# jw007123/hp-Adaptive-Signed-Distance-Field-Octree

Hardware: AMD Instinct MI355X
Metric: Query() Mpts/sec at targetError=1e-5 (union3 field, 10M SplitMix64 pts per GPU, HBM-resident); Create() ms reported as create_ms (higher is better)
Workload: dtype f64

## Files before the change

### hp-adaptive-signed-distance-field-octree_amd/csrc/fit_analytic.hip

```cpp
#include "fit_kernels.hpp"

namespace hpsdf {

HPSDF_FIT_KIND_UNIT(, kFieldAnalytic)

}
```

### hp-adaptive-signed-distance-field-octree_amd/csrc/fit_kernels.hpp

```cpp
#pragma once
#include <hip/hip_runtime.h>

#include <cstdint>

#include "device_types.hpp"
#include "field_glue.hpp"
#include "launch.hpp"

namespace hpsdf {


constexpr int kFitPiece = 8;
#ifndef HPSDF_FIT_MIN_WAVES
#define HPSDF_FIT_MIN_WAVES 4
#endif

__device__ __forceinline__ double fitRowAny(double acc, double a1, const double* __restrict__ tk, double n2,
                                            const double* __restrict__ F, int nq) {
    int k = 0;
    for (; k + 4 <= nq; k += 4) {
        const double f0 = F[k], f1 = F[k + 1], f2 = F[k + 2], f3 = F[k + 3];
        const double t0 = tk[k], t1 = tk[k + 1], t2 = tk[k + 2], t3 = tk[k + 3];
        acc = acc + (a1 * t0 * n2) * f0;
        acc = acc + (a1 * t1 * n2) * f1;
        acc = acc + (a1 * t2 * n2) * f2;
        acc = acc + (a1 * t3 * n2) * f3;
    }
    for (; k < nq; ++k) acc = acc + (a1 * tk[k] * n2) * F[k];
    return acc;
}

template <int KIND, bool CSG, int DEG, int R, bool LEFT>
__device__ __forceinline__ void fitBlockBody(const FitBlock blk, const FitTask* __restrict__ tasks, double* __restrict__ arena,
                                             double* __restrict__ errs, double* __restrict__ mirror,
                                             const DeviceTables* __restrict__ T, const FieldDev& field, const RootMap& rm, double* lds) {
    static_assert(R == 1 || DEG > 0, "cell blocking needs a compile-time degree");
    __shared__ double sNl[13 * 11];
    __shared__ double sRec[26];
    __shared__ int32_t sMeshStack[kFitThreads / 64][kMeshStack];
    __shared__ unsigned char sPosI[KIND == kFieldMesh ? 64 : 4], sPosJK[KIND == kFieldMesh ? 64 : 4];
    const int tid = threadIdx.x;
    const int deg = DEG > 0 ? DEG : (int)blk.degree;
    const int nq = 4 * deg + 1, nq2 = nq * nq, G = blk.nTasks;
    const int rowStart = blk.rowStart, rowEnd = blk.rowEnd, nrows = rowEnd - rowStart;
    const int gl = nq * (nq - 1) / 2;
    const int planes = blk.planesPerChunk;
    const int depth = blk.depth;
    const bool split = blk.split != 0;

    double* sT = lds;
    double* sR = sT + (deg + 1) * nq;
    double* sW = sR + nq;
    double* sC = sW + nq;
    double* sF = sC + 8 * G;

    stageQueryTables(T, sNl, sRec);
    for (int q = tid; q < nq; q += kFitThreads) {
        const double x = T->roots[gl + q];
        sR[q] = x;
        sW[q] = T->weights[gl + q];
        double m2 = 0.0, m1 = 1.0;
        sT[q] = 1.0;
        for (int i = 1; i <= deg; ++i) {
            const double l = T->rec[i][0] * x * m1 - T->rec[i][1] * m2;
            m2 = m1, m1 = l;
            sT[i * nq + q] = l;
        }
    }
    for (int g = tid; g < G; g += kFitThreads) {
        const FitTask& tk = tasks[blk.firstTask + g];
        double sc[3];
        for (int a = 0; a < 3; ++a) {
            sc[a] = (double)(tk.bmax[a] - tk.bmin[a]) * 0.5;
            sC[8 * g + 3 + a] = (double)((tk.bmin[a] + tk.bmax[a]) / 2.0f);
            sC[8 * g + a] = sc[a];
        }
        sC[8 * g + 6] = prod3<LEFT>(sc[0], sc[1], sc[2]);
        sC[8 * g + 7] = __longlong_as_double((long long)tk.sampleOff);
    }
    __syncthreads();

    const bool wide = DEG == 0 && nrows > kFitThreads;
    const int slot = wide ? 0 : tid / nrows;
    const int g2 = slot * R;
    const int r0 = rowStart + (wide ? tid : tid % nrows);
    const int r1 = r0 + kFitThreads;
    const bool act0 = wide ? (r0 < rowEnd) : (tid < ((G + R - 1) / R) * nrows);
    const bool act1 = wide && r1 < rowEnd;
    int i0a = 0, i1a = 0, i2a = 0, i0b = 0, i1b = 0, i2b = 0;
    double n0a = 0, n1a = 0, n2a = 0, n0b = 0, n1b = 0, n2b = 0;
    if (act0) {
        i0a = T->bidx[r0][0], i1a = T->bidx[r0][1], i2a = T->bidx[r0][2];
        n0a = sNl[i0a * 11 + depth], n1a = sNl[i1a * 11 + depth], n2a = sNl[i2a * 11 + depth];
    }
    if (act1) {
        i0b = T->bidx[r1][0], i1b = T->bidx[r1][1], i2b = T->bidx[r1][2];
        n0b = sNl[i0b * 11 + depth], n1b = sNl[i1b * 11 + depth], n2b = sNl[i2b * 11 + depth];
    }
    constexpr int NQF = DEG > 0 ? 4 * DEG + 1 : 1;
    double tkReg[NQF];
    if (DEG > 0) {
#pragma unroll
        for (int k = 0; k < NQF; ++k) tkReg[k] = sT[i2a * nq + k];
    }
    uint32_t meshHint = 0xFFFFFFFFu;
    double acc[R];
#pragma unroll
    for (int r = 0; r < R; ++r) acc[r] = 0.0;
    double acc1 = 0.0;

    const int cellStride = planes * nq2;
    for (int iBase = 0; iBase < nq; iBase += planes) {
        const int np = min(planes, nq - iBase);
        if constexpr (KIND == kFieldMesh) {
            if (tid < nq) {
                int rank = 0;
                for (int b = 0; b < nq; ++b) rank += sR[b] < sR[tid] ? 1 : 0;
                sPosJK[rank] = (unsigned char)tid;
            }
            if (tid >= 64 && tid < 64 + np) {
                const int a = tid - 64;
                int rank = 0;
                for (int b = 0; b < np; ++b) rank += sR[iBase + b] < sR[iBase + a] ? 1 : 0;
                sPosI[rank] = (unsigned char)a;
            }
            __syncthreads();
        }
        if constexpr (KIND != kFieldMesh) {
            const int cols = G * nq2;
            for (int c0 = 0; c0 < cols; c0 += kFitThreads) {
                const int cc = c0 + tid;
                const bool activeS = cc < cols;
                const int ccl = activeS ? cc : cols - 1;
                const int g = ccl / nq2, jk = ccl - g * nq2, j = jk / nq, k = jk - j * nq;
                const double* c = sC + 8 * g;
                const double uy = sR[j] * c[1] + c[4], uz = sR[k] * c[2] + c[5];
                const double wy = uy * rm.bounds[1] + rm.centre[1];
                const double wz = uz * rm.bounds[2] + rm.centre[2];
                const double wj = sW[j], wk = sW[k], c6 = c[6];
                const uint64_t sbase = (uint64_t)__double_as_longlong(c[7]) + (uint64_t)(j * nq + k);
                for (int il = 0; il < np; ++il) {
                    const int i = iBase + il;
                    const double ux = sR[i] * c[0] + c[3];
                    const double wx = ux * rm.bounds[0] + rm.centre[0];
                    const uint64_t sidx = sbase + (uint64_t)(i * nq2);
                    const double fv = activeS ? fieldEvalWorld<KIND, CSG, LEFT>(field, wx, wy, wz, sidx, sNl, sRec, meshHint) : 0.0;
                    if (activeS) {
                        sF[g * cellStride + il * nq2 + jk] = c6 * prod3<LEFT>(sW[i], wj, wk) * fv;
                        if (split) const_cast<double*>(field.samples)[sidx] = fv;
                    }
                }
            }
        } else {
            const int chunkSamples = np * nq2, total = G * chunkSamples;
            const float invChunk = 1.0f / (float)chunkSamples;
            for (int s0 = 0; s0 < total; s0 += kFitThreads) {
                const int s = s0 + tid;
                const bool activeS = s < total;
                const int sc = activeS ? s : total - 1;
                int g = (int)(((float)sc + 0.5f) * invChunk);
                int rem = sc - g * chunkSamples;
                if (rem < 0) {
                    --g;
                    rem += chunkSamples;
                } else if (rem >= chunkSamples) {
                    ++g;
                    rem -= chunkSamples;
                }
                if constexpr (KIND == kFieldMesh) rem = meshSampleOrder(rem, np, nq, sPosI, sPosJK);
                const double* c = sC + 8 * g;
                const int il = rem / nq2, jk = rem - il * nq2, j = jk / nq, k = jk - j * nq, i = iBase + il;
                const double ux = sR[i] * c[0] + c[3], uy = sR[j] * c[1] + c[4], uz = sR[k] * c[2] + c[5];
                const double wx = ux * rm.bounds[0] + rm.centre[0];
                const double wy = uy * rm.bounds[1] + rm.centre[1];
                const double wz = uz * rm.bounds[2] + rm.centre[2];
                const uint64_t sidx = (uint64_t)__double_as_longlong(c[7]) + (uint64_t)((i * nq + j) * nq + k);
                double fv;
                if constexpr (KIND == kFieldMesh) {
                    const double mv = (double)meshSignedDistanceWave(field.mesh, V3{(float)wx, (float)wy, (float)wz}, activeS, meshHint,
                                                                     sMeshStack[tid >> 6]);
                    fv = activeS ? applyCsg<CSG>(field, mv, wx, wy, wz, sNl, sRec) : 0.0;
                } else {
                    fv = activeS ? fieldEvalWorld<KIND, CSG, LEFT>(field, wx, wy, wz, sidx, sNl, sRec, meshHint) : 0.0;
                }
                if (activeS) {
                    sF[g * cellStride + rem] = c[6] * prod3<LEFT>(sW[i], sW[j], sW[k]) * fv;
                    if constexpr (KIND != kFieldMesh)
                        if (split) const_cast<double*>(field.samples)[sidx] = fv;
                }
            }
        }
        __syncthreads();
        if (act0) {
            const double* tj = sT + i1a * nq;
            const double* tk = sT + i2a * nq;
            for (int il = 0; il < np; ++il) {
                const double* F = sF + g2 * cellStride + il * nq2;
                const double a0 = sT[i0a * nq + iBase + il] * n0a;
#ifdef HPSDF_FIT_ROW_UNROLL
#pragma unroll HPSDF_FIT_ROW_UNROLL
#endif
                for (int j = 0; j < nq; ++j) {
                    const double a1 = a0 * tj[j] * n1a;
                    if constexpr (DEG > 0 && DEG <= 5) {
                        double lp[NQF];
#pragma unroll
                        for (int k = 0; k < NQF; ++k) lp[k] = a1 * tkReg[k] * n2a;
#pragma unroll
                        for (int r = 0; r < R; ++r) {
                            const double* Fr = F + r * cellStride + j * nq;
                            double f[NQF];
#pragma unroll
                            for (int k = 0; k < NQF; ++k) f[k] = Fr[k];
#pragma unroll
                            for (int k = 0; k < NQF; ++k) acc[r] = acc[r] + lp[k] * f[k];
                        }
                    } else if constexpr (DEG > 5) {
                        const double* Fr = F + j * nq;
#pragma unroll
                        for (int k0 = 0; k0 < NQF; k0 += kFitPiece) {
                            double lp[kFitPiece], f[kFitPiece];
#pragma unroll
                            for (int k = 0; k < kFitPiece; ++k)
                                if (k0 + k < NQF) f[k] = Fr[k0 + k];
#pragma unroll
                            for (int k = 0; k < kFitPiece; ++k)
                                if (k0 + k < NQF) lp[k] = a1 * tkReg[k0 + k] * n2a;
#pragma unroll
                            for (int k = 0; k < kFitPiece; ++k)
                                if (k0 + k < NQF) acc[0] = acc[0] + lp[k] * f[k];
                        }
                    } else {
                        acc[0] = fitRowAny(acc[0], a1, tk, n2a, F + j * nq, nq);
                    }
                }
            }
        }
        if (act1) {
            const double* tj = sT + i1b * nq;
            const double* tk = sT + i2b * nq;
            for (int il = 0; il < np; ++il) {
                const double* F = sF + il * nq2;
                const double a0 = sT[i0b * nq + iBase + il] * n0b;
                for (int j = 0; j < nq; ++j) {
                    const double a1 = a0 * tj[j] * n1b;
                    acc1 = fitRowAny(acc1, a1, tk, n2b, F + j * nq, nq);
                }
            }
        }
        __syncthreads();
    }

    const bool weighted = blk.weighted != 0;
    const int stashStride = weighted ? rowEnd : nrows, stashBase = weighted ? 0 : rowStart;
    const int outBase = split ? 0 : stashBase;
    if (act0) {
#pragma unroll
        for (int r = 0; r < R; ++r)
            if (g2 + r < G) {
                const uint64_t at = tasks[blk.firstTask + g2 + r].outOff + (r0 - outBase);
                arena[at] = acc[r];
                if (mirror != nullptr) mirror[at] = acc[r];
                sF[(g2 + r) * stashStride + (r0 - stashBase)] = acc[r];
            }
    }
    if (act1) {
        arena[tasks[blk.firstTask].outOff + (r1 - outBase)] = acc1;
        sF[r1 - stashBase] = acc1;
    }
    if (weighted && rowStart > 0) {
        for (int s = tid; s < G * rowStart; s += kFitThreads) {
            const int g = s / rowStart, r = s - g * rowStart;
            const FitTask& tk = tasks[blk.firstTask + g];
            const double v = arena[tk.copyOff + r];
            arena[tk.outOff + r] = v;
            sF[g * stashStride + r] = v;
        }
    }
    __syncthreads();
    for (int g = tid; g < G; g += kFitThreads) {
        const int first = deg > 0 ? (int)T->count[deg - 1] : 0;
        double e = 0.0;
        for (int r = first > rowStart ? first : rowStart; r < rowEnd; ++r)
            if (T->bidx[r][3] == deg) {
                const double c = sF[g * stashStride + (r - stashBase)];
                e = e + c * c;
            }
        errs[tasks[blk.firstTask + g].errSlot] = e;
    }
}

template <int KIND, bool CSG, bool LEFT>
__global__ __launch_bounds__(kFitThreads, HPSDF_FIT_MIN_WAVES) void fit_multi_kernel(const FitBlock* __restrict__ blocks,
                                                                const FitTask* __restrict__ tasks, double* __restrict__ arena,
                                                                double* __restrict__ errs, const DeviceTables* __restrict__ T,
                                                                FieldDev field, RootMap rm, const uint32_t* __restrict__ count,
                                                                uint32_t countValue) {
    extern __shared__ double lds[];
    const uint32_t n = count ? *count : countValue;
    if (blockIdx.x >= n) return;
    const FitBlock blk = blocks[n - 1u - blockIdx.x];
    switch (blk.degree) {
        case 2: fitBlockBody<KIND, CSG, 2, 1, LEFT>(blk, tasks, arena, errs, nullptr, T, field, rm, lds); break;
        case 3: fitBlockBody<KIND, CSG, 3, 1, LEFT>(blk, tasks, arena, errs, nullptr, T, field, rm, lds); break;
        case 4: fitBlockBody<KIND, CSG, 4, 1, LEFT>(blk, tasks, arena, errs, nullptr, T, field, rm, lds); break;
        case 5: fitBlockBody<KIND, CSG, 5, 1, LEFT>(blk, tasks, arena, errs, nullptr, T, field, rm, lds); break;
        case 6: fitBlockBody<KIND, CSG, 6, 1, LEFT>(blk, tasks, arena, errs, nullptr, T, field, rm, lds); break;
        case 7: fitBlockBody<KIND, CSG, 7, 1, LEFT>(blk, tasks, arena, errs, nullptr, T, field, rm, lds); break;
        case 8: fitBlockBody<KIND, CSG, 8, 1, LEFT>(blk, tasks, arena, errs, nullptr, T, field, rm, lds); break;
        default: fitBlockBody<KIND, CSG, 0, 1, LEFT>(blk, tasks, arena, errs, nullptr, T, field, rm, lds); break;
    }
}

template <int KIND, bool CSG, int DEG, int R, bool LEFT>
__global__ __launch_bounds__(kFitThreads, HPSDF_FIT_MIN_WAVES) void fit_kernel(const FitBlock* __restrict__ blocks,
                                                          const FitTask* __restrict__ tasks, double* __restrict__ arena,
                                                          double* __restrict__ errs, double* __restrict__ mirror,
                                                          const DeviceTables* __restrict__ T, FieldDev field, RootMap rm,
                                                          const uint32_t* __restrict__ range) {
    extern __shared__ double lds[];
    uint32_t b = blockIdx.x;
    if (range != nullptr) {
        if (b >= range[1]) return;
        b += range[0];
    }
    fitBlockBody<KIND, CSG, DEG, R, LEFT>(blocks[b], tasks, arena, errs, mirror, T, field, rm, lds);
}

template <int KIND, bool CSG, bool LEFT>
__global__ __launch_bounds__(256) void field_kernel(FieldDev f, const DeviceTables* __restrict__ T,
                                                    const double* __restrict__ xyz, size_t n, double* __restrict__ out) {
    __shared__ double sNl[13 * 11];
    __shared__ double sRec[26];
    stageQueryTables(T, sNl, sRec);
    __syncthreads();
    const size_t stride = (size_t)gridDim.x * blockDim.x;
    uint32_t hint = 0xFFFFFFFFu;
    for (size_t i = (size_t)blockIdx.x * blockDim.x + threadIdx.x; i < n; i += stride)
        out[i] = fieldEvalWorld<KIND, CSG, LEFT>(f, xyz[3 * i], xyz[3 * i + 1], xyz[3 * i + 2], i, sNl, sRec, hint);
}

template <int KIND, bool CSG, bool LEFT>
static void launchFitT(hipStream_t stream, int degree, int cellsPerThread, const FitBlock* dBlocks, uint32_t nBlocks,
                       size_t ldsBytes, const FitTask* dTasks, double* dArena, double* dErrs, double* dMeans,
                       const DeviceTables* dTables, const FieldDev& field, const RootMap& rm, const uint32_t* dRange) {
#define HPSDF_FIT_LAUNCH(D, RR)                                                                                       \
    hipLaunchKernelGGL((fit_kernel<KIND, CSG, D, RR, LEFT>), dim3(nBlocks), dim3(kFitThreads), ldsBytes, stream, dBlocks, \
                       dTasks, dArena, dErrs, dMeans, dTables, field, rm, dRange)
#define HPSDF_FIT_CASE(D)       \
    case D:                     \
        HPSDF_FIT_LAUNCH(D, 1); \
        break;
    if (cellsPerThread != 1 && cellsPerThread != 4) cellsPerThread = 1;
    switch (degree) {
        HPSDF_FIT_CASE(2)
        HPSDF_FIT_CASE(3)
        HPSDF_FIT_CASE(4)
        HPSDF_FIT_CASE(5)
        HPSDF_FIT_CASE(6)
        HPSDF_FIT_CASE(7)
        HPSDF_FIT_CASE(8)
        default:
            HPSDF_FIT_LAUNCH(0, 1);
    }
#undef HPSDF_FIT_CASE
#undef HPSDF_FIT_LAUNCH
}

template <int KIND, bool CSG, bool LEFT>
static void launchFitMultiT(hipStream_t stream, const FitBlock* dBlocks, uint32_t maxBlocks, size_t ldsBytes, const FitTask* dTasks,
                            double* dArena, double* dErrs, const DeviceTables* dTables, const FieldDev& field, const RootMap& rm,
                            const uint32_t* dCount) {
    hipLaunchKernelGGL((fit_multi_kernel<KIND, CSG, LEFT>), dim3(maxBlocks), dim3(kFitThreads), ldsBytes, stream, dBlocks, dTasks, dArena, dErrs,
                       dTables, field, rm, dCount, maxBlocks);
}

template <int KIND, bool CSG, bool LEFT>
static void launchFieldT(hipStream_t stream, const FieldDev& f, const DeviceTables* dTables, const double* dXyz,
                         size_t n, double* dOut) {
    hipLaunchKernelGGL((field_kernel<KIND, CSG, LEFT>), dim3(gridFor(n)), dim3(256), 0, stream, f, dTables, dXyz, n, dOut);
}

#define HPSDF_DISPATCH_FIELD_ORDER(FN, K, C, field, ...)  \
    do {                                                  \
        if ((field).leftAssoc) FN<K, C, true>(__VA_ARGS__); \
        else FN<K, C, false>(__VA_ARGS__);                \
    } while (0)
#define HPSDF_DISPATCH_FIELD(FN, K, field, ...)                                                  \
    do {                                                                                         \
        if ((field).csgOp >= 0) HPSDF_DISPATCH_FIELD_ORDER(FN, K, true, field, __VA_ARGS__);     \
        else HPSDF_DISPATCH_FIELD_ORDER(FN, K, false, field, __VA_ARGS__);                       \
    } while (0)

template <int KIND>
void launchFitKind(hipStream_t stream, int degree, int cellsPerThread, const FitBlock* dBlocks, uint32_t nBlocks, size_t ldsBytes,
                   const FitTask* dTasks, double* dArena, double* dErrs, double* dMirror, const DeviceTables* dTables,
                   const FieldDev& field, const RootMap& rm, const uint32_t* dRange) {
    HPSDF_DISPATCH_FIELD(launchFitT, KIND, field, stream, degree, cellsPerThread, dBlocks, nBlocks, ldsBytes, dTasks, dArena,
                         dErrs, dMirror, dTables, field, rm, dRange);
}
template <int KIND>
void launchFitMultiKind(hipStream_t stream, const FitBlock* dBlocks, uint32_t maxBlocks, size_t ldsBytes, const FitTask* dTasks,
                        double* dArena, double* dErrs, const DeviceTables* dTables, const FieldDev& field, const RootMap& rm,
                        const uint32_t* dCount) {
    HPSDF_DISPATCH_FIELD(launchFitMultiT, KIND, field, stream, dBlocks, maxBlocks, ldsBytes, dTasks, dArena, dErrs, dTables, field, rm, dCount);
}
template <int KIND>
void launchFieldKind(hipStream_t stream, const FieldDev& f, const DeviceTables* dTables, const double* dXyz, size_t n, double* dOut) {
    HPSDF_DISPATCH_FIELD(launchFieldT, KIND, f, stream, f, dTables, dXyz, n, dOut);
}
#undef HPSDF_DISPATCH_FIELD
#undef HPSDF_DISPATCH_FIELD_ORDER

#define HPSDF_FIT_KIND_UNIT(EXTERN, K)                                                                                                 \
    EXTERN template void launchFitKind<K>(hipStream_t, int, int, const FitBlock*, uint32_t, size_t, const FitTask*, double*, double*, \
                                          double*, const DeviceTables*, const FieldDev&, const RootMap&, const uint32_t*);            \
    EXTERN template void launchFitMultiKind<K>(hipStream_t, const FitBlock*, uint32_t, size_t, const FitTask*, double*, double*,      \
                                               const DeviceTables*, const FieldDev&, const RootMap&, const uint32_t*);                \
    EXTERN template void launchFieldKind<K>(hipStream_t, const FieldDev&, const DeviceTables*, const double*, size_t, double*);
HPSDF_FIT_KIND_UNIT(extern, kFieldAnalytic)
HPSDF_FIT_KIND_UNIT(extern, kFieldSamples)
HPSDF_FIT_KIND_UNIT(extern, kFieldMesh)

}
```

Before: 94500.

## Balance deg-2 fit sampling across plane groups and prefetch projection rows

For analytic and CSG fields at degree 2, the sampling phase now splits each column's planes into groups of three and spreads those work units across threads. This is meant to reduce tail imbalance when the column count does not fill the block evenly. The projection loop for R==1 is software-pipelined: the next row of samples and the next basis value are loaded from shared memory before the current row's FMAs, with a scheduling barrier in between to hide LDS latency. Optional timestamp instrumentation is also added behind a macro. The change adds register pressure and repeats the per-unit coordinate setup, and it only affects Create(), not Query().

```diff
diff --git a/hp-adaptive-signed-distance-field-octree_amd/csrc/fit_analytic.hip b/hp-adaptive-signed-distance-field-octree_amd/csrc/fit_analytic.hip
--- a/hp-adaptive-signed-distance-field-octree_amd/csrc/fit_analytic.hip
+++ b/hp-adaptive-signed-distance-field-octree_amd/csrc/fit_analytic.hip
@@ -5,3 +5,10 @@
 HPSDF_FIT_KIND_UNIT(, kFieldAnalytic)
 
 }
+
+#ifdef HPSDF_FIT_STAMPS
+extern "C" __attribute__((visibility("default"))) int hpsdf_debug_fit_stamps(unsigned long long* out, size_t count) {
+    if (hipDeviceSynchronize() != hipSuccess) return 1;
+    return hipMemcpyFromSymbol(out, HIP_SYMBOL(hpsdf::gFitStamps), count * sizeof(unsigned long long)) == hipSuccess ? 0 : 1;
+}
+#endif
diff --git a/hp-adaptive-signed-distance-field-octree_amd/csrc/fit_kernels.hpp b/hp-adaptive-signed-distance-field-octree_amd/csrc/fit_kernels.hpp
--- a/hp-adaptive-signed-distance-field-octree_amd/csrc/fit_kernels.hpp
+++ b/hp-adaptive-signed-distance-field-octree_amd/csrc/fit_kernels.hpp
@@ -13,6 +13,27 @@
 constexpr int kFitPiece = 8;
 #ifndef HPSDF_FIT_MIN_WAVES
 #define HPSDF_FIT_MIN_WAVES 4
+#endif
+
+#ifndef HPSDF_FIT_BALANCE
+#define HPSDF_FIT_BALANCE 1
+#endif
+constexpr int kFitPlaneGroup = 3;
+constexpr bool fitBalanced(int kind, int deg) { return HPSDF_FIT_BALANCE != 0 && kind != kFieldMesh && deg == 2; }
+#ifndef HPSDF_FIT_ROW_AHEAD
+#define HPSDF_FIT_ROW_AHEAD 1
+#endif
+constexpr bool fitRowAhead(int kind, int deg, int r) { return HPSDF_FIT_ROW_AHEAD != 0 && kind != kFieldMesh && deg == 2 && r == 1; }
+
+#ifdef HPSDF_FIT_STAMPS
+constexpr int kFitStampGroups = 4096;
+static __device__ unsigned long long gFitStamps[kFitStampGroups * 4 * 4];
+#define HPSDF_FIT_STAMP(SLOT)                                                                                          \
+    if constexpr (KIND == kFieldAnalytic && DEG == 2)                                                                  \
+        if ((threadIdx.x & 63u) == 0u && blockIdx.x < (unsigned)kFitStampGroups)                                       \
+            gFitStamps[(blockIdx.x * 4u + (threadIdx.x >> 6)) * 4u + (SLOT)] = wall_clock64()
+#else
+#define HPSDF_FIT_STAMP(SLOT)
 #endif
 
 __device__ __forceinline__ double fitRowAny(double acc, double a1, const double* __restrict__ tk, double n2,
@@ -54,6 +75,13 @@
     double* sC = sW + nq;
     double* sF = sC + 8 * G;
 
+#ifdef HPSDF_FIT_STAMPS
+    if constexpr (KIND == kFieldAnalytic && DEG == 2)
+        if ((threadIdx.x & 63u) == 0u && blockIdx.x < (unsigned)kFitStampGroups)
+            gFitStamps[(blockIdx.x * 4u + (threadIdx.x >> 6)) * 4u + 3u] =
+                (unsigned long long)__builtin_amdgcn_s_getreg((31 << 11) | 4) | ((unsigned long long)__builtin_amdgcn_s_getreg((31 << 11) | 20) << 32);
+#endif
+    HPSDF_FIT_STAMP(0u);
     stageQueryTables(T, sNl, sRec);
     for (int q = tid; q < nq; q += kFitThreads) {
         const double x = T->roots[gl + q];
@@ -126,7 +154,38 @@
             }
             __syncthreads();
         }
-        if constexpr (KIND != kFieldMesh) {
+        if constexpr (fitBalanced(KIND, DEG)) {
+            constexpr int kMaxGroups = (NQF + kFitPlaneGroup - 1) / kFitPlaneGroup;
+            const int cols = G * nq2, units = cols * ((np + kFitPlaneGroup - 1) / kFitPlaneGroup);
+            for (int u0 = 0; u0 < units; u0 += kFitThreads) {
+                const int uu = u0 + tid;
+                const bool activeS = uu < units;
+                const int ul = activeS ? uu : units - 1;
+                int pg = 0;
+#pragma unroll
+                for (int q = 1; q < kMaxGroups; ++q) pg += ul >= q * cols ? 1 : 0;
+                const int cc = ul - pg * cols;
+                const int g = cc / nq2, jk = cc - g * nq2, j = jk / nq, k = jk - j * nq;
+                const double* c = sC + 8 * g;
+                const double uy = sR[j] * c[1] + c[4], uz = sR[k] * c[2] + c[5];
+                const double wy = uy * rm.bounds[1] + rm.centre[1];
+                const double wz = uz * rm.bounds[2] + rm.centre[2];
+                const double wj = sW[j], wk = sW[k], c6 = c[6];
+                const uint64_t sbase = (uint64_t)__double_as_longlong(c[7]) + (uint64_t)(j * nq + k);
+                const int ilEnd = min(np, (pg + 1) * kFitPlaneGroup);
+                for (int il = pg * kFitPlaneGroup; il < ilEnd; ++il) {
+                    const int i = iBase + il;
+                    const double ux = sR[i] * c[0] + c[3];
+                    const double wx = ux * rm.bounds[0] + rm.centre[0];
+                    const uint64_t sidx = sbase + (uint64_t)(i * nq2);
+                    const double fv = activeS ? fieldEvalWorld<KIND, CSG, LEFT>(field, wx, wy, wz, sidx, sNl, sRec, meshHint) : 0.0;
+                    if (activeS) {
+                        sF[g * cellStride + il * nq2 + jk] = c6 * prod3<LEFT>(sW[i], wj, wk) * fv;
+                        if (split) const_cast<double*>(field.samples)[sidx] = fv;
+                    }
+                }
+            }
+        } else if constexpr (KIND != kFieldMesh) {
             const int cols = G * nq2;
             for (int c0 = 0; c0 < cols; c0 += kFitThreads) {
                 const int cc = c0 + tid;
@@ -190,8 +249,37 @@
                 }
             }
         }
+        HPSDF_FIT_STAMP(1u);
         __syncthreads();
-        if (act0) {
+        if constexpr (fitRowAhead(KIND, DEG, R)) {
+            if (act0) {
+                const double* tj = sT + i1a * nq;
+                const double* Frow = sF + g2 * cellStride;
+                double fn[NQF];
+#pragma unroll
+                for (int k = 0; k < NQF; ++k) fn[k] = Frow[k];
+                double tjn = tj[0], t0n = sT[i0a * nq + iBase];
+                for (int il = 0; il < np; ++il) {
+                    const bool lastPlane = il + 1 == np;
+                    const double a0 = t0n * n0a;
+                    t0n = sT[i0a * nq + iBase + (lastPlane ? il : il + 1)];
+#pragma unroll
+                    for (int j = 0; j < NQF; ++j) {
+                        double f[NQF];
+#pragma unroll
+                        for (int k = 0; k < NQF; ++k) f[k] = fn[k];
+                        const double a1 = a0 * tjn * n1a;
+                        if (j + 1 < NQF || !lastPlane) Frow += NQF;
+#pragma unroll
+                        for (int k = 0; k < NQF; ++k) fn[k] = Frow[k];
+                        tjn = tj[j + 1 < NQF ? j + 1 : 0];
+                        __builtin_amdgcn_sched_barrier(0);
+#pragma unroll
+                        for (int k = 0; k < NQF; ++k) acc[0] = acc[0] + (a1 * tkReg[k] * n2a) * f[k];
+                    }
+                }
+            }
+        } else if (act0) {
             const double* tj = sT + i1a * nq;
             const double* tk = sT + i2a * nq;
             for (int il = 0; il < np; ++il) {
@@ -248,6 +336,7 @@
                 }
             }
         }
+        HPSDF_FIT_STAMP(2u);
         __syncthreads();
     }
 
```

Result: no change. 94500, median of 4 (+0.0%).
